# jonasBoss/ndarray-interp

Hardware: AMD Instinct MI355X
Metric: interp_array Mpoints/s (queries x lanes), 1D cubic f64 (higher is better)
Workload: dtype f64; 1 GPU; Target: 1D CubicSpline NotAKnot, 4096 knots x 4096 lanes f64, 10000000 queries per GPU in 4 distinct chunks of 2500000 through a 2-slot device-output ring (sorted-unique uniform knots, unsorted uniform in-range queries; output 327.7 GB per step, never copied to the host)

## Files before the change

### ndarray-interp_amd/csrc/float_host.hpp

```cpp

template <class T>
struct Queries {
  const T* a = nullptr;
  const T* b = nullptr;
  int count() const { return b ? 2 : 1; }
  Queries operator+(uint64_t off) const { return {a + off, b ? b + off : nullptr}; }
};

struct FirstFail {
  unsigned long long f0 = NO_FAIL, f1 = NO_FAIL;
  unsigned long long first() const { return std::min(f0, f1); }
  template <class T>
  static FirstFail of(const Workspace& ws, Queries<T> q) {
    return {ws.host_status->first_fail[0], q.b ? ws.host_status->first_fail[1] : NO_FAIL};
  }
};

constexpr size_t ZERO_COPY_LIMIT = 1u << 20;

template <class Plan>
struct RingRun {
  std::unique_lock<std::mutex> own;
  std::vector<void*> slots;
  uint64_t pitch = 0, chunk = 0, cq0 = 0;
  uint32_t n_slots = 0;
  Plan plan0;
  hipStream_t side = nullptr;
};

template <class T, class Impl>
struct FloatEngine {
  Impl& self() { return static_cast<Impl&>(*this); }

  ndi_status report(Queries<T> q, int q_space, FirstFail f, uint64_t index_offset, ndi_oob_info* info) {
    const int axis = f.f0 <= f.f1 ? 0 : 1;
    const unsigned long long ff = axis ? f.f1 : f.f0;
    const T* src = axis ? q.b : q.a;
    T v;
    if (q_space == NDI_MEM_DEVICE) NDI_HIP(hipMemcpy(&v, src + ff, sizeof(T), hipMemcpyDeviceToHost));
    else v = src[ff];
    const ndi_status st = self().failure_status(v);
    if (info) {
      info->index = index_offset + ff;
      info->value = (double)v;
      info->axis = axis;
      info->status = st;
    }
    if (st == NDI_NAN_QUERY) return fail(st, "failed to convert NaN to usize (query %llu)", index_offset + ff);
    return fail(st, "%s = %.17g is not in range", self().axis_name(axis), (double)v);
  }

  ndi_status failure_status(T) { return (self().mode != EX_NO) ? NDI_NAN_QUERY : NDI_OUT_OF_BOUNDS; }

  ndi_status collect(hipStream_t s, Workspace& ws, uint64_t index_offset, ndi_oob_info* info) {
    ws.ensure_status();
    NDI_HIP(hipMemcpyAsync(ws.host_status, ws.sc[0].status.p, sizeof(StatusBlock), hipMemcpyDeviceToHost, s));
    NDI_HIP(hipStreamSynchronize(s));
    ws.pending = false;
    const Queries<T> q{(const T*)ws.last_q, (const T*)ws.last_q2};
    const FirstFail f = FirstFail::of(ws, q);
    if (f.first() == NO_FAIL) return NDI_OK;
    return report(q, ws.last_q_space, f, index_offset, info);
  }

  ndi_status run_finish(void* stream, ndi_oob_info* info) {
    DeviceGuard dg(self().device);
    hipStream_t s = (hipStream_t)stream;
    SpaceLease lease(self().spaces, s);
    Workspace& ws = lease.ws;
    if (!ws.pending) {
      NDI_HIP(hipStreamSynchronize(s));
      return NDI_OK;
    }
    return collect(s, ws, 0, info);
  }

  Queries<T> stage_queries(hipStream_t s, Workspace& ws, Queries<T> q, uint64_t nq, int q_space) {
    if (q_space != NDI_MEM_HOST) return q;
    auto upload = [&](DevBuf& buf, const T* src) -> const T* {
      if (!src) return nullptr;
      buf.reserve(nq * sizeof(T));
      NDI_HIP(hipMemcpyAsync(buf.p, src, nq * sizeof(T), hipMemcpyHostToDevice, s));
      return buf.as<T>();
    };
    const T* a = upload(ws.qdev, q.a);
    return {a, upload(ws.qdev2, q.b)};
  }

  void enqueue_prepass(hipStream_t s, Workspace& ws, Queries<T> q, uint64_t nq) {
    ws.ensure_status();
    reset_status(ws.status.p, s);
    StatusBlock* st = ws.status.as<StatusBlock>();
    T lim[4];
    self().range_limits(lim);
    const unsigned g = (unsigned)std::max<uint64_t>(1, std::min<uint64_t>((nq + BLOCK - 1) / BLOCK, 4096));
    {
      ProfScope ps(s, PC_LOCATE);
      hipLaunchKernelGGL(range_check_kernel<T>, dim3(g), dim3(BLOCK), 0, s, q.a, q.b, nq, lim[0], lim[1], lim[2], lim[3],
                         self().mode, &st->first_fail[0]);
      NDI_HIP(hipGetLastError());
      ps.done();
    }
    NDI_HIP(hipMemcpyAsync(ws.host_status, ws.status.p, sizeof(StatusBlock), hipMemcpyDeviceToHost, s));
  }

  void rows_out(T* dst, uint64_t out_stride, const void* src, uint64_t good) {
    const uint64_t lanes = self().lanes, row_bytes = lanes * sizeof(T);
    if (out_stride == lanes) std::memcpy(dst, src, good * row_bytes);
    else
// ... 32 lines not shown
      }
      if (f.first() != NO_FAIL) return report(q_orig + off, q_space, f, off, info);
    }
    return NDI_OK;
  }

  ndi_status eval_small_zero_copy(hipStream_t s, Workspace& ws, Queries<T> q_host, uint64_t nq, T* out,
                                  uint64_t out_stride, ndi_oob_info* info) {
    const size_t q_bytes = ((nq * sizeof(T)) + 255) & ~(size_t)255, row_bytes = self().lanes * sizeof(T);
    const size_t rows_at = q_host.count() * q_bytes;
    ws.ensure_pin(std::max<size_t>(rows_at + nq * row_bytes, 8ull << 20));
    ws.ensure_status();
    T* pa = reinterpret_cast<T*>(ws.pin);
    T* pb = q_host.b ? reinterpret_cast<T*>((char*)ws.pin + q_bytes) : nullptr;
    T* po = reinterpret_cast<T*>((char*)ws.pin + rows_at);
    std::memcpy(pa, q_host.a, nq * sizeof(T));
    if (pb) std::memcpy(pb, q_host.b, nq * sizeof(T));
    self().small_begin();
    StatusBlock* st = ws.sc[0].status.as<StatusBlock>();
    NDI_HIP(hipMemsetAsync(st, 0xFF, 2 * sizeof(unsigned long long), s));
    const Queries<T> q_pin{ws.pin_device<const T>(pa), pb ? ws.pin_device<const T>(pb) : nullptr};
    self().launch_small(s, st, q_pin, ws.pin_device<T>(po), nq);
    NDI_HIP(hipMemcpyAsync(ws.host_status, st, sizeof(StatusBlock), hipMemcpyDeviceToHost, s));
    NDI_HIP(hipStreamSynchronize(s));
    const FirstFail f = FirstFail::of(ws, q_host);
    const uint64_t good = (f.first() == NO_FAIL) ? nq : (uint64_t)f.first();
    if (good) rows_out(out, out_stride, po, good);
    if (f.first() != NO_FAIL) return report(q_host, NDI_MEM_HOST, f, 0, info);
    return NDI_OK;
  }

  ndi_status eval_body(hipStream_t s, Workspace& ws, Queries<T> q, Queries<T> q_orig, int q_space, uint64_t nq,
                       void* out_, uint64_t out_stride, const ndi_eval_opts& o, ndi_oob_info* info) {
    ws.last_q = q_orig.a;
    ws.last_q2 = q_orig.b;
    ws.last_q_space = q_space;
    ws.last_nq = nq;
    if (o.out_memspace == NDI_MEM_DEVICE) {
      self().enqueue(s, ws, q, nq, (T*)out_, out_stride, o.path, o.flags);
      ws.pending = true;
      if (o.async_launch) return NDI_OK;
      return collect(s, ws, 0, info);
    }
    const uint64_t lanes = self().lanes, row_bytes = lanes * sizeof(T);
    if constexpr (Impl::small_rows)
      if (self().small_rows_fit()) return eval_small_host(s, ws, q, q_orig, q_space, nq, (T*)out_, out_stride, info);
    const uint64_t chunk_q = std::max<uint64_t>(1, std::min<uint64_t>(nq, (256ull << 20) / row_bytes));
    ws.stage.reserve(chunk_q * row_bytes);
    ws.ensure_status();
    for (uint64_t off = 0; off < nq; off += chunk_q) {
      const uint64_t cq = std::min<uint64_t>(chunk_q, nq - off);
      self().enqueue(s, ws, q + off, cq, ws.stage.as<T>(), lanes, o.path, 0);
      NDI_HIP(hipMemcpyAsync(ws.host_status, ws.sc[0].status.p, sizeof(StatusBlock), hipMemcpyDeviceToHost, s));
      NDI_HIP(hipStreamSynchronize(s));
      const FirstFail f = FirstFail::of(ws, q);
      const uint64_t good = (f.first() == NO_FAIL) ? cq : (uint64_t)f.first();
      if (good)
        NDI_HIP(hipMemcpy2D((T*)out_ + off * out_stride, out_stride * sizeof(T), ws.stage.p, row_bytes, row_bytes, good,
                            hipMemcpyDeviceToHost));
      if (f.first() != NO_FAIL) return report(q_orig + off, q_space, f, off, info);
    }
    return NDI_OK;
  }

  ndi_status run_eval(const char* range, Queries<T> q_, uint64_t nq, void* out_, uint64_t out_stride,
                      const ndi_eval_opts* opts, ndi_oob_info* info) {
    DeviceGuard dg(self().device);
    Range rg(range);
    ndi_eval_opts o{};
    if (const ndi_status vs__ = take_opts(opts, o); vs__ != NDI_OK) return vs__;
    hipStream_t s = (hipStream_t)o.stream;
    if (out_stride < self().lanes) return fail(NDI_BAD_ARG, "out_row_stride (%llu) < lanes (%llu)",
                                               (unsigned long long)out_stride, (unsigned long long)self().lanes);
    if (nq == 0) return NDI_OK;
    if (!q_.a || q_.count() != Impl::query_arrays || !out_) return fail(NDI_BAD_ARG, "null query / output pointer");
    SpaceLease lease(self().spaces, s);
    Workspace& ws = lease.ws;
    if (self().zero_copy_fits(nq, o.q_memspace, o.out_memspace))
      return eval_small_zero_copy(s, ws, q_, nq, (T*)out_, out_stride, info);
    const Queries<T> q = stage_queries(s, ws, q_, nq, o.q_memspace);
    return eval_body(s, ws, q, q_, o.q_memspace, nq, out_, out_stride, o, info);
  }

  template <class Plan>
  void ring_begin(hipStream_t s, Workspace& ws, Queries<T> q, uint64_t nq, const ndi_ring_desc* ring, uint64_t stride,
                  const ndi_eval_opts& o, RingRun<Plan>& R) {
    R.n_slots = ring->n_slots;
    R.chunk = ring->chunk_queries;
    R.slots.resize(ring->n_slots);
    R.pitch = stride;
    if (ring->slots) {
      for (uint32_t i = 0; i < ring->n_slots; ++i) R.slots[i] = ring->slots[i];
    } else {
      OwnedRing& ring_own = self().ring_own;
      R.own = std::unique_lock<std::mutex>(ring_own.mu);
      ring_own.ensure(ring->n_slots, ring->chunk_queries, stride * sizeof(T));
      for (uint32_t i = 0; i < ring->n_slots; ++i) R.slots[i] = (char*)ring_own.buf.p + (size_t)i * stride * sizeof(T);
      R.pitch = (uint64_t)ring->n_slots * stride;
    }
    R.side = ring_overlap() ? ws.side_stream() : s;
    for (Scratch& sc : ws.sc) sc.ensure_events();
    NDI_HIP(hipEventRecord(ws.order_event(), s));
    NDI_HIP(hipStreamWaitEvent(R.side, ws.order_event(), 0));
    R.cq0 = std::min<uint64_t>(R.chunk, nq);
    R.plan0 = self().prep(R.side, ws.sc[0], q, R.cq0, (T*)R.slots[0], R.pitch, o.path);
    NDI_HIP(hipEventRecord(ws.sc[0].prep_done, R.side));
  }

  template <class Plan>
  void ring_produce(hipStream_t s, Workspace& ws, Queries<T> q, uint64_t limit, RingRun<Plan>& R,
                    ndi_ring_consumer consume, void* user, const ndi_eval_opts& o, uint64_t q_offset, uint32_t shard) {
    std::vector<hipEvent_t> busy(R.n_slots, nullptr);
    uint64_t k = 0;
    for (uint64_t off = 0; off < limit; off += R.chunk, ++k) {
      const uint64_t cq = std::min<uint64_t>(R.chunk, limit - off);
      const uint32_t slot = (uint32_t)(k % R.n_slots);
      Scratch& sc = ws.sc[k & 1];
      Plan P = R.plan0;
      if (k > 0) {
        if (k >= 2) NDI_HIP(hipStreamWaitEvent(R.side, sc.eval_done, 0));
        P = self().prep(R.side, sc, q + off, cq, (T*)R.slots[slot], R.pitch, o.path, R.side != s);
        NDI_HIP(hipEventRecord(sc.prep_done, R.side));
      }
      NDI_HIP(hipStreamWaitEvent(s, sc.prep_done, 0));
      if (busy[slot]) {
        NDI_HIP(hipStreamWaitEvent(s, busy[slot], 0));
        busy[slot] = nullptr;
      }
      self().launch_eval(s, sc, P);
      NDI_HIP(hipEventRecord(sc.eval_done, s));
      if (consume) {
        ndi_ring_chunk c{};
        c.index = k; c.q_begin = q_offset + off; c.q_count = cq; c.out = R.slots[slot]; c.row_stride = R.pitch;
        c.slot = slot; c.shard = shard; c.stream = (void*)s;
        busy[slot] = (hipEvent_t)consume(user, &c);
      }
    }
    NDI_HIP(hipStreamSynchronize(s));
    NDI_HIP(hipStreamSynchronize(R.side));
    for (hipEvent_t e : busy)
      if (e) NDI_HIP(hipEventSynchronize(e));
    ws.pending = false;
  }

  ndi_status run_ring(const char* range, Queries<T> q_, uint64_t nq, const ndi_ring_desc* ring, ndi_ring_consumer consume,
                      void* user, const ndi_eval_opts* opts, ndi_oob_info* info) {
    DeviceGuard dg(self().device);
    ndi_eval_opts o{};
    if (const ndi_status vs__ = take_opts(opts, o); vs__ != NDI_OK) return vs__;
    hipStream_t s = (hipStream_t)o.stream;
    uint64_t stride = 0;
    ndi_status rs = check_ring_desc(ring, self().lanes, &stride);
    if (rs != NDI_OK) return rs;
    if (nq == 0) return NDI_OK;
    if (!q_.a || q_.count() != Impl::query_arrays) return fail(NDI_BAD_ARG, "null query pointer");
    Range rg(range);
    SpaceLease lease(self().spaces, s);
    Workspace& ws = lease.ws;
    const Queries<T> q = stage_queries(s, ws, q_, nq, o.q_memspace);
    enqueue_prepass(s, ws, q, nq);
    RingRun<typename Impl::Plan> R;
    ring_begin(s, ws, q, nq, ring, stride, o, R);
    NDI_HIP(hipStreamSynchronize(s));
    const FirstFail f = FirstFail::of(ws, q);
    const uint64_t limit = f.first() == NO_FAIL ? nq : std::min<uint64_t>(nq, f.first());
    ring_produce(s, ws, q, limit, R, consume, user, o, 0, 0);
    if (f.first() == NO_FAIL) return NDI_OK;
    return report(q_, o.q_memspace, f, 0, info);
  }

  void trim_front() {
    self().spaces.trim();
    if constexpr (Impl::ring) {
      std::lock_guard<std::mutex> g(self().ring_own.mu);
      self().ring_own.clear();
    }
  }
};
```

### ndarray-interp_amd/csrc/kernels.hpp

```cpp
#pragma once
#include <hip/hip_runtime.h>
#include <stdint.h>

#include <type_traits>

namespace ndi {

constexpr unsigned long long NO_FAIL = ~0ull;
constexpr int BLOCK = 256;

enum ExtrapMode : int { EX_NO = 0, EX_YES = 1, EX_PERIODIC = 2 };
enum Strat : int { ST_LINEAR = 0, ST_CUBIC = 1 };

struct StatusBlock {
  unsigned long long first_fail[2];
  unsigned long long n_valid;
  unsigned long long periodic_mismatch;
  unsigned int ticket;
  unsigned int reserved;
};

#ifdef NDI_BOUNDS
__device__ unsigned long long g_ndi_bounds[4];
__device__ __forceinline__ unsigned long long ndi_bounds_fail(int code, int line, unsigned long long idx,
// ... 1928 lines not shown
  const uint64_t q_begin = (uint64_t)blockIdx.x * slice;
  uint64_t q_end = q_begin + slice;
  if (q_end > nq) q_end = nq;
  for (uint64_t qi = q_begin + threadIdx.x; qi < q_end; qi += BLOCK) {
    const uint32_t i = NDI_CHK(idx[qi], nb, BC_BIN);
    const uint32_t pos = NDI_CHK(atomicAdd(&cur[i], 1u), nq, BC_POSITION);
    rec[pos] = make_rec<T>((uint32_t)qi, i, sval[qi]);
  }
}

template <class T, int STRAT, int U, int CQ, bool NT = true, bool FULL = false>
__global__ __launch_bounds__(BLOCK) void eval_bucketed_kernel(Eval1Args<T> A) {
  constexpr int VN = Wide<T>::N;
  using V = typename VecT<T, VN>::type;
  __shared__ uint32_t s_q[CQ];
  __shared__ uint32_t s_i[CQ];
  __shared__ T s_s[CQ];
  const uint64_t LV = A.lanes / VN;
  const uint32_t seg_vecs = BLOCK * U;
  const uint32_t segs = (uint32_t)((LV + seg_vecs - 1) / seg_vecs);
  const unsigned long long n_valid = A.nq;
  unsigned long long limit = A.status->first_fail[0];
  if (limit > A.nq) limit = A.nq;
  const uint64_t nchunks = (n_valid + CQ - 1) / CQ;
  const uint64_t per = (nchunks + 7) / 8;
  const uint64_t run = A.run ? A.run : 1;
  const uint64_t runs_per_xcd = (per + run - 1) / run;
  for (uint32_t seg = blockIdx.y; seg < segs; seg += gridDim.y) {
    const uint64_t v0 = (uint64_t)seg * seg_vecs + threadIdx.x;
    for (uint64_t vb = blockIdx.x; vb < runs_per_xcd * 8; vb += gridDim.x) {
      const uint64_t xcd = vb & 7u;
      const uint64_t c_begin = xcd * per + (vb >> 3) * run;
      uint64_t c_end = c_begin + run;
      if (c_end > (xcd + 1) * per) c_end = (xcd + 1) * per;
      if (c_end > nchunks) c_end = nchunks;
      V ryl[U], ryr[U], ra[U], rb[U];
      uint32_t cur = 0xffffffffu;
      for (uint64_t chunk = c_begin; chunk < c_end; ++chunk) {
        const uint64_t p0 = chunk * CQ;
        const uint32_t cnt = (n_valid - p0 < (uint64_t)CQ) ? (uint32_t)(n_valid - p0) : (uint32_t)CQ;
        __syncthreads();
        for (uint32_t j = threadIdx.x; j < cnt; j += BLOCK) {
          const uint4 r = A.rec[p0 + j];
          s_q[j] = r.x;
          s_i[j] = r.y;
          s_s[j] = rec_value(r, T(0));
        }
        __syncthreads();
        auto emit = [&](uint32_t i, uint32_t qi, T sj) {
          const RowCoef<T, STRAT> c = row_coef<T, STRAT>(A.knots, i, sj, sj);
          V* o = reinterpret_cast<V*>(A.out + (uint64_t)qi * A.out_stride);
#pragma unroll
          for (int u = 0; u < U; ++u) {
            const uint64_t v = v0 + (uint64_t)u * BLOCK;
            if (FULL || v < LV) store_stream<NT>(o + v, row_point<T, STRAT, V>(c, ryl[u], ryr[u], ra[u], rb[u]));
          }
        };
        for (uint32_t j = 0; j < cnt;) {
          const uint32_t i = NDI_CHK((uint32_t)__builtin_amdgcn_readfirstlane((int)s_i[j]), A.n_int, BC_INTERVAL);
          const uint32_t qi = NDI_CHK((uint32_t)__builtin_amdgcn_readfirstlane((int)s_q[j]), A.nq, BC_QUERY);
          if (qi >= limit) { ++j; continue; }
          if (i != cur) {
            cur = i;
            const V* yl = reinterpret_cast<const V*>(A.data + (uint64_t)i * A.lanes);
            const V* yr = yl + LV;
            const V* pa = reinterpret_cast<const V*>(A.ca + (uint64_t)i * A.lanes);
            const V* pb = reinterpret_cast<const V*>(A.cb + (uint64_t)i * A.lanes);
#pragma unroll
            for (int u = 0; u < U; ++u) {
              const uint64_t v = v0 + (uint64_t)u * BLOCK;
              if (FULL || v < LV) {
                ryl[u] = yl[v];
                ryr[u] = yr[v];
                if (STRAT == ST_CUBIC) {
                  ra[u] = pa[v];
                  rb[u] = pb[v];
                }
              }
            }
          }
          emit(i, qi, s_s[j]);
          ++j;
        }
      }
    }
  }
}

template <class T, int STRAT, int G, int CQ, bool NT = true>
__global__ __launch_bounds__(BLOCK) void eval_bucketed_short_kernel(Eval1Args<T> A) {
  constexpr int VN = Wide<T>::N;
  using V = typename VecT<T, VN>::type;
  constexpr uint32_t NG = BLOCK / G;
  constexpr uint32_t WQ = NG * CQ;
  __shared__ uint32_t s_q[WQ];
  __shared__ uint32_t s_i[WQ];
  __shared__ T s_s[WQ];
  const uint32_t LV = (uint32_t)(A.lanes / VN);
  const uint32_t g = threadIdx.x / G, v = threadIdx.x % G;
  const bool vlive = v < LV;
  const unsigned long long n_valid = A.nq;
  unsigned long long limit = A.status->first_fail[0];
  if (limit > A.nq) limit = A.nq;
  const uint64_t nchunks = (n_valid + WQ - 1) / WQ;
  const uint64_t per = (nchunks + 7) / 8;
  V ryl = V(0), ryr = V(0), ra = V(0), rb = V(0);
  uint32_t cur = 0xffffffffu;
  for (uint64_t vb = blockIdx.x; vb < per * 8; vb += gridDim.x) {
    const uint64_t chunk = (vb & 7u) * per + (vb >> 3);
    if (chunk >= nchunks) continue;
    const uint64_t p0 = chunk * WQ;
    const uint32_t cnt = (n_valid - p0 < (uint64_t)WQ) ? (uint32_t)(n_valid - p0) : WQ;
    __syncthreads();
    for (uint32_t j = threadIdx.x; j < cnt; j += BLOCK) {
      const uint4 r = A.rec[p0 + j];
      s_q[j] = r.x;
      s_i[j] = r.y;
      s_s[j] = rec_value(r, T(0));
    }
    __syncthreads();
    const uint32_t j0 = g * CQ;
    const uint32_t j1 = (j0 + CQ < cnt) ? j0 + CQ : cnt;
    for (uint32_t j = j0; j < j1; ++j) {
      const uint32_t i = NDI_CHK(s_i[j], A.n_int, BC_INTERVAL);
      const uint32_t qi = NDI_CHK(s_q[j], A.nq, BC_QUERY);
      if (qi >= limit) continue;
      const T sj = s_s[j];
      if (i != cur) {
        cur = i;
        if (vlive) {
          const V* yl = reinterpret_cast<const V*>(A.data + (uint64_t)i * A.lanes);
          ryl = yl[v];
          ryr = yl[LV + v];
          if (STRAT == ST_CUBIC) {
            ra = reinterpret_cast<const V*>(A.ca + (uint64_t)i * A.lanes)[v];
            rb = reinterpret_cast<const V*>(A.cb + (uint64_t)i * A.lanes)[v];
          }
        }
      }
      const RowCoef<T, STRAT> c = row_coef<T, STRAT>(A.knots, i, sj, sj);
      V* o = reinterpret_cast<V*>(A.out + (uint64_t)qi * A.out_stride);
      if (vlive) store_stream<NT>(o + v, row_point<T, STRAT, V>(c, ryl, ryr, ra, rb));
    }
  }
}

template <class T>
struct Eval2Args {
  const T* xk;
  const T* yk;
  const T* data;
  const T* qx;
  const T* qy;
  const uint32_t* xi;
  const uint32_t* yi;
  T* out;
  uint64_t nx, ny, lanes, out_stride, nq;
  uint64_t row_cells, cell_elems;
  const StatusBlock* status;
  const uint4* rec_i;
  const T* rec_q;
  const uint32_t* bin_start;
  uint32_t nb, ts, nty, chunk;
  const uint32_t* chunk_bin;
  int debug;
  uint32_t rvm_full, rvm_edge;
// ... 2405 lines not shown
```

### ndarray-interp_amd/csrc/ndinterp_api.hip

```cpp
#include <dlfcn.h>

#include <algorithm>
#include <atomic>
#include <chrono>
#include <condition_variable>
#include <cmath>
#include <cstdlib>
#include <cstring>
#include <functional>
#include <limits>
#include <map>
#include <memory>
#include <mutex>
#include <set>
#include <shared_mutex>
#include <stdexcept>
#include <thread>
#include <unordered_map>
#include <utility>
#include <vector>

#include "common.hpp"
#include "host_logic.hpp"
#include "kernels.hpp"
// ... 335 lines not shown
      const T scale = best_scale;
      m = best_m;
      cnt.assign(m, 0);
      best_k = 0;
      for (uint64_t i = 0; i < n; ++i) {
        T f = (knots[i] - k0) * scale;
        f = std::fmax(f, T(0));
        f = std::fmin(f, T(m - 1u));
        best_k = std::max(best_k, ++cnt[(uint32_t)f]);
      }
      std::vector<uint16_t> lut((size_t)m + 2 + 6, (uint16_t)n);
      uint32_t run = 0;
      for (uint32_t b = 0; b < m; ++b) {
        lut[b] = (uint16_t)run;
        run += cnt[b];
      }
      const size_t bytes = (((size_t)(m + 2) / 2) * 4 + 15) & ~(size_t)15;
      try {
        maybe_fail_lazy_alloc(__LINE__);
        self->dlut_buf.reserve(std::max(bytes, lut.size() * sizeof(uint16_t)));
        NDI_HIP(hipMemcpy(self->dlut_buf.p, lut.data(), lut.size() * sizeof(uint16_t), hipMemcpyHostToDevice));
      } catch (const HipFailure&) {
        (void)hipGetLastError();
        self->dlut_buf.release();
        return;
      }
      self->dlut = DenseLut<T>{self->dlut_buf.template as<uint16_t>(), m, best_k, scale};
      self->dlut_bytes = bytes;
      self->dense_ok = true;
    });
  }

  DevBuf lut_buf;
  BucketIndex<T> bidx{nullptr, 0, T(0)};
  size_t lut_bytes = 0;
  void build_bucket_index(const T* knots, uint64_t n, bool guess_is_exact) {
    bidx = BucketIndex<T>{nullptr, 0, T(0)};
    lut_bytes = 0;
    if (guess_is_exact || n <= 64 || n > 65535) return;
    uint32_t m = 1;
    while (m < 2 * n) m *= 2;
    const T k0 = knots[0], kn = knots[n - 1];
    const T scale = T(m) / (kn - k0);
    if (!(scale > T(0)) || !std::isfinite((double)scale)) return;
    std::vector<uint16_t> lut(m + 2 + 6, 0);
    std::vector<uint32_t> cnt(m, 0);
    for (uint64_t i = 0; i < n; ++i) cnt[bucket_of<T>(knots[i], k0, scale, m)]++;
    uint32_t run = 0;
    for (uint32_t b = 0; b < m; ++b) {
      lut[b] = (uint16_t)run;
      run += cnt[b];
    }
    for (size_t b = m; b < lut.size(); ++b) lut[b] = (uint16_t)n;
    const size_t bytes = (((size_t)(m + 2) / 2) * 4 + 15) & ~(size_t)15;
    lut_buf.reserve(std::max(bytes, lut.size() * sizeof(uint16_t)));
    NDI_HIP(hipMemcpy(lut_buf.p, lut.data(), lut.size() * sizeof(uint16_t), hipMemcpyHostToDevice));
    bidx = BucketIndex<T>{lut_buf.as<uint16_t>(), m, scale};
    lut_bytes = bytes;
  }
};

constexpr uint64_t MAX_KNOTS = (1ull << 31) - 1;
constexpr size_t LDS_STAGE_LIMIT = 150 * 1024;
constexpr size_t FUSED_LDS_LIMIT = 160 * 1024;

struct Scratch {
  DevBuf idx, idx2, t, perm, counts, cursor, hist, status, recq, chunkbin;
  DevBuf perm2, recq2, chist, cursor2;
  hipEvent_t prep_done = nullptr, eval_done = nullptr;
  Scratch() = default;
  Scratch(const Scratch&) = delete;
  Scratch& operator=(const Scratch&) = delete;
  ~Scratch() {
    if (prep_done) (void)hipEventDestroy(prep_done);
    if (eval_done) (void)hipEventDestroy(eval_done);
  }
  void ensure_events() {
    if (!prep_done) NDI_HIP(hipEventCreateWithFlags(&prep_done, hipEventDisableTiming));
    if (!eval_done) NDI_HIP(hipEventCreateWithFlags(&eval_done, hipEventDisableTiming));
  }
};

struct Workspace {
  Scratch sc[2];
  DevBuf status, qdev, qdev2, stage;
  StatusBlock* host_status = nullptr;
  void* pin = nullptr;
  void* pin_dev = nullptr;
  size_t pin_bytes = 0;
  hipStream_t side = nullptr;
  hipEvent_t ev = nullptr;
  uint64_t last_nq = 0;
  const void* last_q = nullptr;
  const void* last_q2 = nullptr;
  int last_q_space = NDI_MEM_DEVICE;
  bool pending = false;
  int users = 0;
  uint64_t last_use = 0;
  ~Workspace() {
    if (side) (void)hipStreamDestroy(side);
    if (ev) (void)hipEventDestroy(ev);
    if (host_status) (void)hipHostFree(host_status);
    if (pin) (void)hipHostFree(pin);
  }
  void ensure_pin(size_t need) {
    if (need <= pin_bytes) return;
    if (pin) (void)hipHostFree(pin);
    pin = nullptr;
    pin_dev = nullptr;
    pin_bytes = 0;
    NDI_HIP(hipHostMalloc(&pin, need, hipHostMallocMapped | hipHostMallocPortable));
    NDI_HIP(hipHostGetDevicePointer(&pin_dev, pin, 0));
    pin_bytes = need;
  }
  template <class U>
  U* pin_device(const void* host_ptr) const {
    return reinterpret_cast<U*>((char*)pin_dev + ((const char*)host_ptr - (const char*)pin));
  }
  void ensure_status() {
    status.reserve(sizeof(StatusBlock));
    for (Scratch& s : sc) s.status.reserve(sizeof(StatusBlock));
    if (!host_status) NDI_HIP(hipHostMalloc((void**)&host_status, sizeof(StatusBlock), hipHostMallocDefault));
  }
  hipStream_t side_stream() {
    if (!side) {
      int lo = 0, hi = 0;
      NDI_HIP(hipDeviceGetStreamPriorityRange(&lo, &hi));
      NDI_HIP(hipStreamCreateWithPriority(&side, hipStreamNonBlocking, hi));
    }
    return side;
  }
  hipEvent_t order_event() {
    if (!ev) NDI_HIP(hipEventCreateWithFlags(&ev, hipEventDisableTiming));
    return ev;
  }
};

struct SpaceSet {
  static constexpr size_t MAX_IDLE = 16;
  std::mutex mu;
  std::map<SpaceKey, std::unique_ptr<Workspace>> map;
  uint64_t tick = 0;

  Workspace& acquire(hipStream_t s) {
    std::lock_guard<std::mutex> g(mu);
    auto& slot = map[SpaceKey{s, std::this_thread::get_id()}];
    if (!slot) slot.reset(new Workspace());
    slot->users++;
    slot->last_use = ++tick;
    evict_locked(MAX_IDLE);
    return *slot;
  }
  void release(Workspace& w) {
    std::lock_guard<std::mutex> g(mu);
    w.users--;
  }
  void evict_locked(size_t keep) {
    for (;;) {
      size_t idle = 0;
      auto victim = map.end();
      for (auto it = map.begin(); it != map.end(); ++it) {
        if (it->second->users != 0 || it->second->pending) continue;
        ++idle;
        if (victim == map.end() || it->second->last_use < victim->second->last_use) victim = it;
      }
      if (idle <= keep || victim == map.end()) return;
      map.erase(victim);
    }
  }
  void trim() {
    std::lock_guard<std::mutex> g(mu);
    evict_locked(0);
  }
  size_t size() {
    std::lock_guard<std::mutex> g(mu);
    return map.size();
  }
};

struct SpaceLease {
  SpaceSet& set;
  Workspace& ws;
  SpaceLease(SpaceSet& st, hipStream_t s) : set(st), ws(st.acquire(s)) {}
  ~SpaceLease() { set.release(ws); }
  SpaceLease(const SpaceLease&) = delete;
  SpaceLease& operator=(const SpaceLease&) = delete;
};

struct OwnedRing {
  std::mutex mu;
  DevBuf buf;
  void ensure(uint32_t n, size_t chunk_rows, size_t stride_bytes) { buf.reserve((size_t)n * chunk_rows * stride_bytes); }
  void clear() { buf.release(); }
};

template <class T, class K, class A>
static void launch1(hipStream_t s, int cat, dim3 grid, dim3 block, size_t shmem, K kernel, const A& args) {
  ProfScope ps(s, cat);
  hipLaunchKernelGGL(kernel, grid, block, shmem, s, args);
  NDI_HIP(hipGetLastError());
  ps.done();
}

static void reset_status(void* status, hipStream_t s) {
// ... 63 lines not shown
  A.t = t;
  A.first_fail = first_fail;
  A.mode = mode;
  A.stage_lds = pyr.lds_bytes <= LDS_STAGE_LIMIT ? 1 : 0;
  size_t shmem = A.stage_lds ? ((pyr.lds_bytes + 15) & ~(size_t)15) : 0;
  uint64_t blocks = hist ? std::min<uint64_t>((nq + 2047) / 2048, GROUP_MAX_BLOCKS)
                         : std::min<uint64_t>((nq + 1023) / 1024, 2048);
  blocks = std::max<uint64_t>(blocks, 1);
  A.bx = BucketIndex<T>{nullptr, 0, T(0)};
  constexpr int lut_env = 1;
  if (lut_env && A.stage_lds && nq >= 4096) pyr.ensure_bucket_index();
  if (lut_env && A.stage_lds && pyr.lut_bytes && nq >= 4096 &&
      shmem + pyr.lut_bytes + (hist ? (size_t)nb * 4 : 0) <= LDS_STAGE_LIMIT) {
    A.bx = pyr.bidx;
    shmem += pyr.lut_bytes;
    const size_t total = shmem + (hist ? (size_t)nb * 4 : 0);
    blocks = std::min<uint64_t>(blocks, (uint64_t)cu_count() * std::max<size_t>(1, (160 * 1024) / total));
  }
  A.bx32 = BucketIndex32<T>{nullptr, 0, T(0)};
  if (lut_env && !A.stage_lds && nq >= 4096) {
    pyr.ensure_bucket_index32();
    A.bx32 = pyr.bidx32;
  }
  if (hist) shmem += (size_t)nb * 4;
  const unsigned threads = beside_eval ? 256u : threads_for_lds(shmem);
  uint64_t slice = (nq + blocks - 1) / blocks;
  slice = (slice + threads - 1) / threads * threads;
  blocks = (nq + slice - 1) / slice;
  A.slice = slice;
  A.hist = hist;
  A.nb = nb;
  allow_dynamic_lds(reinterpret_cast<const void*>(&locate_kernel<T, true, LOCATE_QB>), (int)LDS_STAGE_LIMIT);
  allow_dynamic_lds(reinterpret_cast<const void*>(&locate_kernel<T, false, LOCATE_QB>), (int)LDS_STAGE_LIMIT);
  allow_dynamic_lds(reinterpret_cast<const void*>(&locate_kernel<T, true, 1>), (int)LDS_STAGE_LIMIT);
  allow_dynamic_lds(reinterpret_cast<const void*>(&locate_kernel<T, false, 1>), (int)LDS_STAGE_LIMIT);
  if (slice_out) *slice_out = slice;
  if (blocks_out) *blocks_out = (uint32_t)blocks;
  const bool deep = slice / threads >= 16;
  if (A.stage_lds && deep) launch1<T>(s, PC_LOCATE, dim3((unsigned)blocks), dim3(threads), shmem, locate_kernel<T, true, LOCATE_QB>, A);
  else if (A.stage_lds) launch1<T>(s, PC_LOCATE, dim3((unsigned)blocks), dim3(threads), shmem, locate_kernel<T, true, 1>, A);
  else if (deep) launch1<T>(s, PC_LOCATE, dim3((unsigned)blocks), dim3(threads), shmem, locate_kernel<T, false, LOCATE_QB>, A);
  else launch1<T>(s, PC_LOCATE, dim3((unsigned)blocks), dim3(threads), shmem, locate_kernel<T, false, 1>, A);
}

static inline bool aligned16(const void* p) { return (reinterpret_cast<uintptr_t>(p) & 15u) == 0; }

static ndi_status take_opts(const ndi_eval_opts* opts, ndi_eval_opts& o) {
  o = ndi_eval_opts{};
  if (!opts) return NDI_OK;
  o = *opts;
  constexpr int32_t KNOWN = NDI_EVAL_FRESH_OUTPUT | NDI_EVAL_ROWS_AFTER_ERROR_UNSPECIFIED;
  if (o.flags & ~KNOWN) return fail(NDI_BAD_ARG, "ndi_eval_opts.flags has unknown bits (0x%x): built against another header version?", (unsigned)o.flags);
  if (o.reserved != 0) return fail(NDI_BAD_ARG, "ndi_eval_opts.reserved must be 0 (got %d): built against another header version?", (int)o.reserved);
  if (o.flags & NDI_EVAL_ROWS_AFTER_ERROR_UNSPECIFIED) o.flags |= NDI_EVAL_FRESH_OUTPUT;
  return NDI_OK;
}

struct ShortKnobs {
  int mode = 0, unr = 2, tb = 0, lds = -1, wgs = 0, cq = 64, rowb = 1024, pack = -1, maxlv = 256;
  static int env(const char* name, int dflt) {
    const char* e = std::getenv(name);
    return e && *e ? std::atoi(e) : dflt;
  }
  static ShortKnobs read() {
    ShortKnobs k;
    k.mode = env("NDI_SHORT_MODE", k.mode);
    k.unr = env("NDI_FUSED_UNR", k.unr);
    k.tb = env("NDI_FUSED_TB", k.tb);
    k.lds = env("NDI_FUSED_LDS", k.lds);
    k.wgs = env("NDI_FUSED_WGS", k.wgs);
    k.cq = env("NDI_SHORT_CQ", k.cq);
    k.rowb = env("NDI_SHORT_ROWB", k.rowb);
    k.pack = env("NDI_FUSED_PACK", k.pack);
    return k;
  }
};
static ShortKnobs short_knobs() {
  static const bool live = std::getenv("NDI_TUNE_LIVE") != nullptr;
  static const ShortKnobs once = ShortKnobs::read();
  return live ? ShortKnobs::read() : once;
}

static constexpr bool ring_overlap() { return true; }

static ndi_status check_ring_desc(const ndi_ring_desc* ring, uint64_t lanes, uint64_t* stride) {
  if (!ring || ring->n_slots == 0 || ring->chunk_queries == 0)
    return fail(NDI_BAD_ARG, "ring needs n_slots >= 1 and chunk_queries >= 1");
  *stride = ring->row_stride ? ring->row_stride : lanes;
  if (*stride < lanes) return fail(NDI_BAD_ARG, "ring row_stride (%llu) < lanes (%llu)",
                                   (unsigned long long)*stride, (unsigned long long)lanes);
  if (ring->slots)
    for (uint32_t i = 0; i < ring->n_slots; ++i)
      if (!ring->slots[i]) return fail(NDI_BAD_ARG, "ring slot %u is null", i);
  return NDI_OK;
}

#include "float_host.hpp"

struct BuildClock {
  bool on;
  std::chrono::steady_clock::time_point t0, last;
  BuildClock() : on(std::getenv("NDI_BUILD_TIMING") != nullptr), t0(std::chrono::steady_clock::now()), last(t0) {}
  void mark(const char* what) {
    if (!on) return;
    const auto now = std::chrono::steady_clock::now();
    std::fprintf(stderr, "[ndi build] %-28s +%8.3f ms  (%8.3f)\n", what,
                 std::chrono::duration<double, std::milli>(now - last).count(),
                 std::chrono::duration<double, std::milli>(now - t0).count());
    last = now;
  }
};

struct BuildScratch {
  std::map<int, std::pair<void*, size_t>> dev;
  void* pin = nullptr;
  size_t pin_bytes = 0;
  void* device_buf(int device, size_t need) {
    auto& e = dev[device];
    if (need > e.second) {
      if (e.first) (void)hipFree(e.first);
      e = {nullptr, 0};
      const size_t cap = std::max<size_t>(need, 64 * 1024);
      NDI_HIP(hipMalloc(&e.first, cap));
      e.second = cap;
    }
    return e.first;
  }
  void* pinned(size_t need) {
    if (need > pin_bytes) {
      if (pin) (void)hipHostFree(pin);
      pin = nullptr;
      pin_bytes = 0;
      const size_t cap = std::max<size_t>(need, 64 * 1024);
      NDI_HIP(hipHostMalloc(&pin, cap, hipHostMallocPortable));
      pin_bytes = cap;
    }
    return pin;
  }
};
static BuildScratch& build_scratch() {
  static thread_local BuildScratch* p = nullptr;
  if (!p) p = new BuildScratch();
  return *p;
}

static uint64_t fnv1a(uint64_t h, const void* p, size_t bytes) {
  const unsigned char* b = static_cast<const unsigned char*>(p);
  for (size_t i = 0; i < bytes; ++i) h = (h ^ b[i]) * 0x100000001b3ull;
  return h;
}
constexpr uint64_t FNV_SEED = 0xcbf29ce484222325ull;

struct Interp1DBase {
  virtual ~Interp1DBase() = default;
  virtual uint64_t signature() const = 0;
  int dtype = 0, device = 0;
  uint64_t lanes = 0;
  virtual ndi_status eval(const void* q, uint64_t nq, void* out, uint64_t out_stride,
                          const ndi_eval_opts* opts, ndi_oob_info* info) = 0;
  virtual ndi_status finish(void* stream, ndi_oob_info* info) = 0;
  virtual ndi_status coefficients(void* a_out, void* b_out, int memspace) = 0;
  virtual ndi_status eval_ring(const void* q, uint64_t nq, const ndi_ring_desc* ring, ndi_ring_consumer consume,
                               void* user, const ndi_eval_opts* opts, ndi_oob_info* info) = 0;
  virtual ndi_status trim() = 0;
  virtual uint64_t scratch_sets() = 0;
  virtual ndi_status clone_to(int dev, Interp1DBase** out) = 0;
// ... 920 lines not shown
    A.t = sc.t.as<T>();
    A.out = P.out;
    A.lanes = lanes;
    A.out_stride = P.out_stride;
    A.nq = nq;
    A.status = st;
    A.n_int = (uint32_t)(n - 1);
#ifdef NDI_BOUNDS
    if (ShortKnobs::env("NDI_BOUNDS_SELFTEST", 0)) A.n_int = 1;
#endif
    constexpr int VN = Wide<T>::N;
    const uint64_t LV = P.LV;
    if (P.kind == Plan1::BUCKETED) {
      A.rec = sc.perm.as<uint4>();
      constexpr int CQ = 128;
      const int U = LV >= 2048 ? 8 : (LV >= 1024 ? 4 : (LV >= 512 ? 2 : 1));
      const uint64_t segs = (LV + (uint64_t)BLOCK * U - 1) / ((uint64_t)BLOCK * U);
      const uint64_t per_xcd = ((nq + CQ - 1) / CQ + 7) / 8;
      A.run = BUCKETED_RUN;
      const uint64_t runs_per_xcd = (per_xcd + A.run - 1) / A.run;
      const unsigned gx = (unsigned)std::max<uint64_t>(8, std::min<uint64_t>(runs_per_xcd * 8, 65528));
      dim3 grid(gx, (unsigned)std::min<uint64_t>(segs, 64));
      const bool full = LV % ((uint64_t)BLOCK * U) == 0;
#define NDI_BK(ST, UU)                                                                                      \
  do {                                                                                                      \
    if (full) launch1<T>(s, PC_EVAL, grid, dim3(BLOCK), 0, eval_bucketed_kernel<T, ST, UU, CQ, true, true>, A); \
    else launch1<T>(s, PC_EVAL, grid, dim3(BLOCK), 0, eval_bucketed_kernel<T, ST, UU, CQ, true, false>, A);   \
  } while (0)
      if (strategy == NDI_CUBIC_SPLINE) {
        if (U == 8) NDI_BK(ST_CUBIC, 8); else if (U == 4) NDI_BK(ST_CUBIC, 4);
        else if (U == 2) NDI_BK(ST_CUBIC, 2); else NDI_BK(ST_CUBIC, 1);
      } else {
        if (U == 8) NDI_BK(ST_LINEAR, 8); else if (U == 4) NDI_BK(ST_LINEAR, 4);
        else if (U == 2) NDI_BK(ST_LINEAR, 2); else NDI_BK(ST_LINEAR, 1);
      }
#undef NDI_BK
      return;
    }
    if (P.kind == Plan1::BUCKETED_SHORT) {
      A.rec = sc.perm.as<uint4>();
      uint32_t G = 8;
      while (G < LV) G *= 2;
      const int CQ = P.s_cq == 16 ? 16 : 64;
      const uint64_t wq = (uint64_t)(BLOCK / G) * CQ;
      const uint64_t per_xcd = ((nq + wq - 1) / wq + 7) / 8;
      const unsigned gx = (unsigned)std::max<uint64_t>(8, std::min<uint64_t>(per_xcd * 8, 65528));
#define NDI_BS(ST, GG)                                                                                          \
  do {                                                                                                          \
    if (CQ == 16) launch1<T>(s, PC_EVAL, dim3(gx), dim3(BLOCK), 0, eval_bucketed_short_kernel<T, ST, GG, 16>, A); \
    else launch1<T>(s, PC_EVAL, dim3(gx), dim3(BLOCK), 0, eval_bucketed_short_kernel<T, ST, GG, 64>, A);          \
  } while (0)
#define NDI_BSG(ST)                                                                   \
  do {                                                                                \
    if (G == 8) NDI_BS(ST, 8); else if (G == 16) NDI_BS(ST, 16);                      \
    else if (G == 32) NDI_BS(ST, 32); else if (G == 64) NDI_BS(ST, 64);               \
    else if (G == 128) NDI_BS(ST, 128); else NDI_BS(ST, 256);                         \
  } while (0)
      if (strategy == NDI_CUBIC_SPLINE) NDI_BSG(ST_CUBIC); else NDI_BSG(ST_LINEAR);
#undef NDI_BSG
#undef NDI_BS
      return;
    }
    if (P.kind == Plan1::ROWS) {
      const uint64_t segs = (LV + BLOCK - 1) / BLOCK;
      const unsigned gx = (unsigned)std::max<uint64_t>(1, std::min<uint64_t>(nq, 65536));
      dim3 grid(gx, (unsigned)std::min<uint64_t>(segs, 64));
      if (strategy == NDI_CUBIC_SPLINE) launch1<T>(s, PC_EVAL, grid, dim3(BLOCK), 0, eval_rows_kernel<T, ST_CUBIC, 1>, A);
      else launch1<T>(s, PC_EVAL, grid, dim3(BLOCK), 0, eval_rows_kernel<T, ST_LINEAR, 1>, A);
      return;
    }
    const uint32_t tile_q = (uint32_t)std::max<uint64_t>(1, 1024 / std::max<uint64_t>(LV, 1));
    const uint64_t ntiles = (nq + tile_q - 1) / tile_q;
    const unsigned gx = (unsigned)std::max<uint64_t>(1, std::min<uint64_t>(ntiles, 16384));
    ProfScope ps(s, PC_EVAL);
    if (strategy == NDI_CUBIC_SPLINE) {
      if (P.vec_ok) hipLaunchKernelGGL((eval_flat_kernel<T, ST_CUBIC, VN>), dim3(gx), dim3(BLOCK), 0, s, A, tile_q);
      else hipLaunchKernelGGL((eval_flat_kernel<T, ST_CUBIC, 1>), dim3(gx), dim3(BLOCK), 0, s, A, tile_q);
    } else {
      if (P.vec_ok) hipLaunchKernelGGL((eval_flat_kernel<T, ST_LINEAR, VN>), dim3(gx), dim3(BLOCK), 0, s, A, tile_q);
      else hipLaunchKernelGGL((eval_flat_kernel<T, ST_LINEAR, 1>), dim3(gx), dim3(BLOCK), 0, s, A, tile_q);
    }
    NDI_HIP(hipGetLastError());
    ps.done();
  }

  void launch_fused(hipStream_t s, Scratch& sc, const Plan1& P) {
    EvalFusedArgs<T> F{};
    F.pyr = pyr.view;
    F.bx = P.f_lut ? pyr.bidx : BucketIndex<T>{nullptr, 0, T(0)};
    F.data = data.as<T>();
    F.ca = ca.as<T>();
    F.cb = cb.as<T>();
    F.ck = ck.as<T>();
    F.bx32 = P.f_tlds == 3 ? pyr.bidx32 : BucketIndex32<T>{nullptr, 0, T(0)};
    F.rec_stride = (uint32_t)P.LV;
    if (P.f_pack) {
      F.data = packed.as<T>();
      F.ca = packed.as<T>() + 2 * lanes;
      F.cb = packed.as<T>() + 3 * lanes;
      F.rec_stride = (uint32_t)P.LV * (strategy == NDI_CUBIC_SPLINE ? 4u : 2u);
    }
    F.q = P.q;
    F.out = P.out;
    F.nq = P.nq;
    F.out_stride = P.out_stride;
    F.lanes = (uint32_t)lanes;
    F.lv = (uint32_t)P.LV;
    F.lv_magic = F.lv >= 2 ? (uint32_t)(((1ull << 32) + F.lv - 1) / F.lv) : 0u;
    F.mode = mode;
    F.first_fail = &sc.status.as<StatusBlock>()->first_fail[0];
    F.check = P.l_check ? 1 : 0;
    F.debug = 0;
#ifdef NDI_TUNING
    F.debug = ShortKnobs::env("NDI_FUSED_DEBUG", 0);
#endif
    constexpr int VN = Wide<T>::N;
    const dim3 grid(P.f_grid), block(P.f_tb);
    if (P.f_sorted) {
      if (std::getenv("NDI_TRACE_PLAN"))
        std::fprintf(stderr, "[ndi plan] fused sorted lut=%d tb=%u grid=%u lds=%zu prepass=%d\n", (int)P.f_lut, P.f_tb, P.f_grid,
                     P.f_lds, P.l_check ? 0 : 1);
#define NDI_FSK(ST, VEC, QPT)                                                                          \
  do {                                                                                                 \
    auto kern = eval_fused_sorted_kernel<T, ST, VEC, 512, QPT>;                                        \
    allow_dynamic_lds(reinterpret_cast<const void*>(kern), (int)(FUSED_LDS_LIMIT - 256));              \
    launch1<T>(s, PC_EVAL, grid, dim3(512), P.f_lds, kern, F);                                         \
  } while (0)
      if (strategy == NDI_CUBIC_SPLINE) { if (P.vec_ok) NDI_FSK(ST_CUBIC, VN, 8); else NDI_FSK(ST_CUBIC, 1, 8); }
      else { if (P.vec_ok) NDI_FSK(ST_LINEAR, VN, 4); else NDI_FSK(ST_LINEAR, 1, 4); }
#undef NDI_FSK
      return;
    }
    if (std::getenv("NDI_TRACE_PLAN"))
      std::fprintf(stderr, "[ndi plan] fused tables=%s lut=%d pack=%d unr=%d tb=%u grid=%u lds=%zu prepass=%d\n",
                   P.f_tlds == 2 ? "lds{y,k}" : (P.f_tlds == 1 ? "lds{y,a,b}" : (P.f_tlds == 3 ? "memory,knots=global" : "memory")),
                   (int)P.f_lut, (int)P.f_pack,
                   P.f_unr, P.f_tb, P.f_grid, P.f_lds, P.l_check ? 0 : 1);
#define NDI_FU(ST, VEC, UNR, TB, TL)                                                                   \
  do {                                                                                                 \
    auto kern = eval_fused_kernel<T, ST, VEC, UNR, TB, TL>;                                            \
    allow_dynamic_lds(reinterpret_cast<const void*>(kern), (int)FUSED_LDS_LIMIT);                      \
    launch1<T>(s, PC_EVAL, grid, block, P.f_lds, kern, F);                                             \
  } while (0)
#define NDI_FU_TB(ST, VEC, UNR, TL)                                      \
  do {                                                                   \
    if (P.f_tb == 1024) NDI_FU(ST, VEC, UNR, 1024, TL);                  \
    else if (P.f_tb == 512) NDI_FU(ST, VEC, UNR, 512, TL);               \
    else NDI_FU(ST, VEC, UNR, 256, TL);                                  \
  } while (0)
#define NDI_FU_UNR(ST, VEC, TL)                                          \
  do {                                                                   \
    if (P.f_unr == 4) NDI_FU_TB(ST, VEC, 4, TL);                         \
    else if (P.f_unr == 1) NDI_FU_TB(ST, VEC, 1, TL);                    \
    else NDI_FU_TB(ST, VEC, 2, TL);                                      \
  } while (0)
#define NDI_FU_ST(VEC, TL)                                                              \
  do {                                                                                  \
    if (strategy == NDI_CUBIC_SPLINE) NDI_FU_UNR(ST_CUBIC, VEC, TL);                    \
    else NDI_FU_UNR(ST_LINEAR, VEC, TL);                                                \
  } while (0)
    if (P.f_tlds == 3) {
      if (strategy == NDI_CUBIC_SPLINE) { if (P.vec_ok) NDI_FU(ST_CUBIC, VN, 2, 256, 3); else NDI_FU(ST_CUBIC, 1, 2, 256, 3); }
      else { if (P.vec_ok) NDI_FU(ST_LINEAR, VN, 2, 256, 3); else NDI_FU(ST_LINEAR, 1, 2, 256, 3); }
    } else if (P.vec_ok) {
      if (P.f_tlds == 2) NDI_FU_UNR(ST_CUBIC, VN, 2);
      else if (P.f_tlds) NDI_FU_ST(VN, 1);
// ... 2790 lines not shown
```

Baseline: 850,000 Mpoints/s.

## Group consecutive ring chunks into one bucketed eval kernel launch

Adds a grouped bucketed evaluation kernel that processes up to four ring chunks in one launch, interleaving their query tiles across XCD-striped blocks. The ring producer now preps several chunks ahead with more scratch sets and launches them together when their plans are bucketed and compatible. The intent is to cut per-chunk launch and tail-idle costs and keep the GPU saturated across chunk boundaries. In exchange it needs more scratch memory and more prep done up front. Grouping falls back to single-chunk launches once a consumer returns a busy event.

```diff
diff --git a/ndarray-interp_amd/csrc/float_host.hpp b/ndarray-interp_amd/csrc/float_host.hpp
--- a/ndarray-interp_amd/csrc/float_host.hpp
+++ b/ndarray-interp_amd/csrc/float_host.hpp
@@ -22,9 +22,13 @@
 struct RingRun {
   std::unique_lock<std::mutex> own;
   std::vector<void*> slots;
-  uint64_t pitch = 0, chunk = 0, cq0 = 0;
+  uint64_t pitch = 0, chunk = 0;
   uint32_t n_slots = 0;
-  Plan plan0;
+  uint32_t wmax = 1;
+  bool narrow_first = false;
+  uint32_t n_sets = 2;
+  uint64_t prepped = 0;
+  std::vector<Plan> plans;
   hipStream_t side = nullptr;
 };
 
@@ -223,6 +227,18 @@
     return eval_body(s, ws, q, q_, o.q_memspace, nq, out_, out_stride, o, info);
   }
 
+  static constexpr bool ring_groups = false;
+
+  template <class Plan>
+  void ring_prep(hipStream_t s, Workspace& ws, Queries<T> q, uint64_t k, uint64_t cq, RingRun<Plan>& R, int path,
+                 bool beside_eval) {
+    Scratch& sc = ws.sc[k % R.n_sets];
+    if (k >= R.n_sets) NDI_HIP(hipStreamWaitEvent(R.side, sc.eval_done, 0));
+    R.plans[k % R.n_sets] = self().prep(R.side, sc, q + k * R.chunk, cq, (T*)R.slots[k % R.n_slots], R.pitch, path,
+                                        beside_eval);
+    NDI_HIP(hipEventRecord(sc.prep_done, R.side));
+  }
+
   template <class Plan>
   void ring_begin(hipStream_t s, Workspace& ws, Queries<T> q, uint64_t nq, const ndi_ring_desc* ring, uint64_t stride,
                   const ndi_eval_opts& o, RingRun<Plan>& R) {
@@ -240,42 +256,76 @@
       R.pitch = (uint64_t)ring->n_slots * stride;
     }
     R.side = ring_overlap() ? ws.side_stream() : s;
-    for (Scratch& sc : ws.sc) sc.ensure_events();
+    const int mode = Impl::ring_groups ? ring_group_mode() : 0;
+    R.wmax = mode ? std::min<uint32_t>({R.n_slots, (uint32_t)RING_GROUP_MAX, Workspace::MAX_SETS / 2}) : 1u;
+    R.narrow_first = mode == 2;
+    R.n_sets = 2 * R.wmax;
+    R.plans.assign(R.n_sets, Plan{});
+    for (uint32_t i = 0; i < R.n_sets; ++i) ws.sc[i].ensure_events();
     NDI_HIP(hipEventRecord(ws.order_event(), s));
     NDI_HIP(hipStreamWaitEvent(R.side, ws.order_event(), 0));
-    R.cq0 = std::min<uint64_t>(R.chunk, nq);
-    R.plan0 = self().prep(R.side, ws.sc[0], q, R.cq0, (T*)R.slots[0], R.pitch, o.path);
-    NDI_HIP(hipEventRecord(ws.sc[0].prep_done, R.side));
+    uint64_t first = 1;
+    if constexpr (Impl::ring_groups)
+      if (!R.narrow_first) first = std::min<uint64_t>(R.wmax, (nq + R.chunk - 1) / R.chunk);
+    for (R.prepped = 0; R.prepped < first;) {
+      const uint64_t k = R.prepped++;
+      ring_prep(s, ws, q, k, std::min<uint64_t>(R.chunk, nq - k * R.chunk), R, o.path, false);
+      if constexpr (Impl::ring_groups)
+        if (!self().groupable(R.plans[k])) break;
+    }
   }
 
   template <class Plan>
   void ring_produce(hipStream_t s, Workspace& ws, Queries<T> q, uint64_t limit, RingRun<Plan>& R,
                     ndi_ring_consumer consume, void* user, const ndi_eval_opts& o, uint64_t q_offset, uint32_t shard) {
     std::vector<hipEvent_t> busy(R.n_slots, nullptr);
-    uint64_t k = 0;
-    for (uint64_t off = 0; off < limit; off += R.chunk, ++k) {
-      const uint64_t cq = std::min<uint64_t>(R.chunk, limit - off);
-      const uint32_t slot = (uint32_t)(k % R.n_slots);
-      Scratch& sc = ws.sc[k & 1];
-      Plan P = R.plan0;
-      if (k > 0) {
-        if (k >= 2) NDI_HIP(hipStreamWaitEvent(R.side, sc.eval_done, 0));
-        P = self().prep(R.side, sc, q + off, cq, (T*)R.slots[slot], R.pitch, o.path, R.side != s);
-        NDI_HIP(hipEventRecord(sc.prep_done, R.side));
-      }
-      NDI_HIP(hipStreamWaitEvent(s, sc.prep_done, 0));
-      if (busy[slot]) {
-        NDI_HIP(hipStreamWaitEvent(s, busy[slot], 0));
-        busy[slot] = nullptr;
-      }
-      self().launch_eval(s, sc, P);
-      NDI_HIP(hipEventRecord(sc.eval_done, s));
-      if (consume) {
+    const uint64_t nchunks = (limit + R.chunk - 1) / R.chunk;
+    auto count = [&](uint64_t k) { return std::min<uint64_t>(R.chunk, limit - k * R.chunk); };
+    bool solo = R.wmax == 1;
+    uint64_t prepped = R.prepped;
+    for (uint64_t k = 0; k < nchunks;) {
+      uint32_t want = solo || (R.narrow_first && k == 0) ? 1u : (uint32_t)std::min<uint64_t>(R.wmax, nchunks - k);
+      uint32_t w = 0;
+      while (w < want) {
+        if (k + w >= prepped) {
+          ring_prep(s, ws, q, k + w, count(k + w), R, o.path, R.side != s);
+          prepped = k + w + 1;
+        }
+        bool joins = w == 0;
+        if constexpr (Impl::ring_groups) joins = joins || (self().groupable(R.plans[k % R.n_sets]) &&
+                                                          self().groupable(R.plans[(k + w) % R.n_sets]));
+        if (!joins) break;
+        ++w;
+      }
+      Scratch* sets[RING_GROUP_MAX];
+      Plan plans[RING_GROUP_MAX];
+      for (uint32_t i = 0; i < w; ++i) {
+        sets[i] = &ws.sc[(k + i) % R.n_sets];
+        plans[i] = R.plans[(k + i) % R.n_sets];
+        NDI_HIP(hipStreamWaitEvent(s, sets[i]->prep_done, 0));
+        const uint32_t slot = (uint32_t)((k + i) % R.n_slots);
+        if (busy[slot]) {
+          NDI_HIP(hipStreamWaitEvent(s, busy[slot], 0));
+          busy[slot] = nullptr;
+        }
+      }
+      bool grouped = false;
+      if constexpr (Impl::ring_groups)
+        if (self().groupable(plans[0])) {
+          self().launch_eval_group(s, sets, plans, w);
+          grouped = true;
+        }
+      if (!grouped) self().launch_eval(s, *sets[0], plans[0]);
+      for (uint32_t i = 0; i < w; ++i) NDI_HIP(hipEventRecord(sets[i]->eval_done, s));
+      for (uint32_t i = 0; i < w && consume; ++i) {
+        const uint32_t slot = (uint32_t)((k + i) % R.n_slots);
         ndi_ring_chunk c{};
-        c.index = k; c.q_begin = q_offset + off; c.q_count = cq; c.out = R.slots[slot]; c.row_stride = R.pitch;
-        c.slot = slot; c.shard = shard; c.stream = (void*)s;
+        c.index = k + i; c.q_begin = q_offset + (k + i) * R.chunk; c.q_count = count(k + i); c.out = R.slots[slot];
+        c.row_stride = R.pitch; c.slot = slot; c.shard = shard; c.stream = (void*)s;
         busy[slot] = (hipEvent_t)consume(user, &c);
-      }
+        if (busy[slot]) solo = true;
+      }
+      k += w;
     }
     NDI_HIP(hipStreamSynchronize(s));
     NDI_HIP(hipStreamSynchronize(R.side));
diff --git a/ndarray-interp_amd/csrc/kernels.hpp b/ndarray-interp_amd/csrc/kernels.hpp
--- a/ndarray-interp_amd/csrc/kernels.hpp
+++ b/ndarray-interp_amd/csrc/kernels.hpp
@@ -2034,6 +2034,117 @@
           emit(i, qi, s_s[j]);
           ++j;
         }
+      }
+    }
+  }
+}
+
+constexpr int RING_GROUP_MAX = 4;
+template <class T>
+struct EvalGroupArgs {
+  Eval1Args<T> A;
+  const uint4* rec[RING_GROUP_MAX];
+  uint64_t nq[RING_GROUP_MAX];
+  T* out[RING_GROUP_MAX];
+  const StatusBlock* status[RING_GROUP_MAX];
+  uint32_t width;
+};
+
+template <class T, int STRAT, int U, int CQ, bool NT = true, bool FULL = false>
+__global__ __launch_bounds__(BLOCK) void eval_bucketed_group_kernel(EvalGroupArgs<T> G) {
+  constexpr int VN = Wide<T>::N;
+  using V = typename VecT<T, VN>::type;
+  __shared__ uint32_t s_q[CQ];
+  __shared__ uint32_t s_i[CQ];
+  __shared__ T s_s[CQ];
+  const Eval1Args<T>& A = G.A;
+  const uint64_t LV = A.lanes / VN;
+  const uint32_t seg_vecs = BLOCK * U;
+  const uint32_t segs = (uint32_t)((LV + seg_vecs - 1) / seg_vecs);
+  const uint32_t width = G.width;
+  uint64_t nmax = 0;
+#pragma unroll
+  for (int w = 0; w < RING_GROUP_MAX; ++w) {
+    const uint64_t n_w = (uint32_t)w < width ? (G.nq[w] + CQ - 1) / CQ : 0;
+    if (n_w > nmax) nmax = n_w;
+  }
+  const uint64_t n_virtual = nmax * width;
+  const uint64_t per = (n_virtual + 7) / 8;
+  for (uint32_t seg = blockIdx.y; seg < segs; seg += gridDim.y) {
+    const uint64_t v0 = (uint64_t)seg * seg_vecs + threadIdx.x;
+    for (uint64_t vb = blockIdx.x; vb < per * 8; vb += gridDim.x) {
+      const uint64_t xcd = vb & 7u;
+      const uint64_t vi = xcd * per + (vb >> 3);
+      if (vi >= n_virtual) continue;
+      const uint64_t rnd = vi / width;
+      const uint32_t c = (uint32_t)(vi - rnd * width);
+      const uint4* rec = G.rec[0];
+      uint64_t nq = G.nq[0];
+      T* out = G.out[0];
+      const StatusBlock* status = G.status[0];
+#pragma unroll
+      for (int w = 1; w < RING_GROUP_MAX; ++w)
+        if (c == (uint32_t)w) {
+          rec = G.rec[w];
+          nq = G.nq[w];
+          out = G.out[w];
+          status = G.status[w];
+        }
+      const uint64_t n_c = (nq + CQ - 1) / CQ;
+      uint64_t chunk = rnd;
+      if (n_c != nmax) {
+        chunk = rnd * n_c / nmax;
+        if ((rnd + 1) * n_c / nmax == chunk) continue;
+      }
+      const unsigned long long n_valid = nq;
+      unsigned long long limit = status->first_fail[0];
+      if (limit > nq) limit = nq;
+      V ryl[U], ryr[U], ra[U], rb[U];
+      uint32_t cur = 0xffffffffu;
+      const uint64_t p0 = chunk * CQ;
+      const uint32_t cnt = (n_valid - p0 < (uint64_t)CQ) ? (uint32_t)(n_valid - p0) : (uint32_t)CQ;
+      __syncthreads();
+      for (uint32_t j = threadIdx.x; j < cnt; j += BLOCK) {
+        const uint4 r = rec[p0 + j];
+        s_q[j] = r.x;
+        s_i[j] = r.y;
+        s_s[j] = rec_value(r, T(0));
+      }
+      __syncthreads();
+      auto emit = [&](uint32_t i, uint32_t qi, T sj) {
+        const RowCoef<T, STRAT> cf = row_coef<T, STRAT>(A.knots, i, sj, sj);
+        V* o = reinterpret_cast<V*>(out + (uint64_t)qi * A.out_stride);
+#pragma unroll
+        for (int u = 0; u < U; ++u) {
+          const uint64_t v = v0 + (uint64_t)u * BLOCK;
+          if (FULL || v < LV) store_stream<NT>(o + v, row_point<T, STRAT, V>(cf, ryl[u], ryr[u], ra[u], rb[u]));
+        }
+      };
+      for (uint32_t j = 0; j < cnt;) {
+        const uint32_t i = NDI_CHK((uint32_t)__builtin_amdgcn_readfirstlane((int)s_i[j]), A.n_int, BC_INTERVAL);
+        const uint32_t qi = NDI_CHK((uint32_t)__builtin_amdgcn_readfirstlane((int)s_q[j]), nq, BC_QUERY);
+        if (qi >= limit) { ++j; continue; }
+        if (i != cur) {
+          cur = i;
+          const V* yl = reinterpret_cast<const V*>(A.data + (uint64_t)i * A.lanes);
+          const V* yr = yl + LV;
+          const V* pa = reinterpret_cast<const V*>(A.ca + (uint64_t)i * A.lanes);
+          const V* pb = reinterpret_cast<const V*>(A.cb + (uint64_t)i * A.lanes);
+#pragma unroll
+          for (int u = 0; u < U; ++u) {
+            const uint64_t v = v0 + (uint64_t)u * BLOCK;
+            if (FULL || v < LV) {
+              ryl[u] = yl[v];
+              ryr[u] = yr[v];
+              if (STRAT == ST_CUBIC) {
+                ra[u] = pa[v];
+                rb[u] = pb[v];
+              }
+            }
+          }
+        }
+        emit(i, qi, s_s[j]);
+        ++j;
       }
     }
   }
diff --git a/ndarray-interp_amd/csrc/ndinterp_api.hip b/ndarray-interp_amd/csrc/ndinterp_api.hip
--- a/ndarray-interp_amd/csrc/ndinterp_api.hip
+++ b/ndarray-interp_amd/csrc/ndinterp_api.hip
@@ -441,7 +441,8 @@
 };
 
 struct Workspace {
-  Scratch sc[2];
+  static constexpr uint32_t MAX_SETS = 8;
+  Scratch sc[MAX_SETS];
   DevBuf status, qdev, qdev2, stage;
   StatusBlock* host_status = nullptr;
   void* pin = nullptr;
@@ -478,7 +479,7 @@
   }
   void ensure_status() {
     status.reserve(sizeof(StatusBlock));
-    for (Scratch& s : sc) s.status.reserve(sizeof(StatusBlock));
+    for (int i = 0; i < 2; ++i) sc[i].status.reserve(sizeof(StatusBlock));
     if (!host_status) NDI_HIP(hipHostMalloc((void**)&host_status, sizeof(StatusBlock), hipHostMallocDefault));
   }
   hipStream_t side_stream() {
@@ -708,6 +709,14 @@
 }
 
 static constexpr bool ring_overlap() { return true; }
+
+constexpr int RING_GROUP_DEFAULT = 1;
+static int ring_group_mode() {
+  static const bool live = std::getenv("NDI_TUNE_LIVE") != nullptr;
+  static const int once = ShortKnobs::env("NDI_RING_GROUP", RING_GROUP_DEFAULT);
+  const int m = live ? ShortKnobs::env("NDI_RING_GROUP", RING_GROUP_DEFAULT) : once;
+  return m >= 0 && m <= 2 ? m : RING_GROUP_DEFAULT;
+}
 
 static ndi_status check_ring_desc(const ndi_ring_desc* ring, uint64_t lanes, uint64_t* stride) {
   if (!ring || ring->n_slots == 0 || ring->chunk_queries == 0)
@@ -1794,6 +1803,60 @@
     }
     NDI_HIP(hipGetLastError());
     ps.done();
+  }
+
+  static constexpr bool ring_groups = true;
+  static bool groupable(const Plan1& P) { return P.kind == Plan1::BUCKETED; }
+
+  void launch_eval_group(hipStream_t s, Scratch* const* sc, const Plan1* P, uint32_t w) {
+    if (std::getenv("NDI_TRACE_PLAN"))
+      std::fprintf(stderr, "[ndi plan] ring bucketed L=%llu lv=%llu width=%u nq=%llu\n", (unsigned long long)lanes,
+                   (unsigned long long)P[0].LV, w, (unsigned long long)P[0].nq);
+    if (w == 1) {
+      launch_eval(s, *sc[0], P[0]);
+      return;
+    }
+    if (w > (uint32_t)RING_GROUP_MAX) throw HipFailure{hipErrorInvalidValue, "launch_eval_group: group too wide", __LINE__};
+    EvalGroupArgs<T> G{};
+    G.A.knots = pyr.view.lv0;
+    G.A.data = data.as<T>();
+    G.A.ca = ca.as<T>();
+    G.A.cb = cb.as<T>();
+    G.A.lanes = lanes;
+    G.A.out_stride = P[0].out_stride;
+    G.A.n_int = (uint32_t)(n - 1);
+    G.width = w;
+    constexpr int CQ = 128;
+    uint64_t nmax = 0;
+    for (uint32_t i = 0; i < w; ++i) {
+      if (!groupable(P[i]) || P[i].out_stride != P[0].out_stride || P[i].LV != P[0].LV)
+        throw HipFailure{hipErrorInvalidValue, "launch_eval_group: plans of one group differ", __LINE__};
+      G.rec[i] = sc[i]->perm.as<uint4>();
+      G.nq[i] = P[i].nq;
+      G.out[i] = P[i].out;
+      G.status[i] = sc[i]->status.as<StatusBlock>();
+      nmax = std::max<uint64_t>(nmax, (P[i].nq + CQ - 1) / CQ);
+    }
+    const uint64_t LV = P[0].LV;
+    const int U = LV >= 2048 ? 8 : (LV >= 1024 ? 4 : (LV >= 512 ? 2 : 1));
+    const uint64_t segs = (LV + (uint64_t)BLOCK * U - 1) / ((uint64_t)BLOCK * U);
+    const uint64_t per_xcd = (nmax * w + 7) / 8;
+    const unsigned gx = (unsigned)std::max<uint64_t>(8, std::min<uint64_t>(per_xcd * 8, 65528));
+    dim3 grid(gx, (unsigned)std::min<uint64_t>(segs, 64));
+    const bool full = LV % ((uint64_t)BLOCK * U) == 0;
+#define NDI_BG(ST, UU)                                                                                            \
+  do {                                                                                                            \
+    if (full) launch1<T>(s, PC_EVAL, grid, dim3(BLOCK), 0, eval_bucketed_group_kernel<T, ST, UU, CQ, true, true>, G); \
+    else launch1<T>(s, PC_EVAL, grid, dim3(BLOCK), 0, eval_bucketed_group_kernel<T, ST, UU, CQ, true, false>, G);   \
+  } while (0)
+    if (strategy == NDI_CUBIC_SPLINE) {
+      if (U == 8) NDI_BG(ST_CUBIC, 8); else if (U == 4) NDI_BG(ST_CUBIC, 4);
+      else if (U == 2) NDI_BG(ST_CUBIC, 2); else NDI_BG(ST_CUBIC, 1);
+    } else {
+      if (U == 8) NDI_BG(ST_LINEAR, 8); else if (U == 4) NDI_BG(ST_LINEAR, 4);
+      else if (U == 2) NDI_BG(ST_LINEAR, 2); else NDI_BG(ST_LINEAR, 1);
+    }
+#undef NDI_BG
   }
 
   void launch_fused(hipStream_t s, Scratch& sc, const Plan1& P) {
```

Result: faster. 863,300 Mpoints/s (median of 6 runs) (+1.6%).
